# q-optimize/c3

Hardware: AMD Instinct MI355X
Metric: full-gate propagators/s (higher is better)
Workload: dtype c128

## Files before the change

### c3_amd/csrc/c3p_smalld.hip

```cpp
#include <type_traits>

#include <cstdlib>
#include "c3p_common.h"
#include "c3p_kernels.h"
#include "c3p_smalld.h"

#ifdef C3P_SMALLD_PART
#define C3P_SMALLD_HAS(p) (C3P_SMALLD_PART == (p))
#else
#define C3P_SMALLD_HAS(p) 1
#endif

extern __shared__ __attribute__((aligned(16))) double c3p_sd_lds[];

namespace {

template <int D>
struct SD {
  static constexpr int NBI = (D + 1) / 2;
  static constexpr int NJ = (D + 3) / 4;
  static constexpr int W = 4 * NJ + 1;
  static constexpr int MAT = 4 * NBI * W;
  static constexpr int IMG = ((MAT - 12 + 31) / 32) * 32 + 12;
};

__device__ __forceinline__ double mfma4(double a, double b, double c) {
  return __builtin_amdgcn_mfma_f64_4x4x4f64(a, b, c, 0, 0, 0);
}

__device__ __forceinline__ double readfirstlane_f64(double v) {
  int lo = __double2loint(v), hi = __double2hiint(v);
  lo = __builtin_amdgcn_readfirstlane(lo);
  hi = __builtin_amdgcn_readfirstlane(hi);
  return __hiloint2double(hi, lo);
}

typedef __attribute__((address_space(3))) const volatile double c3p_lds_cvd;
__device__ __forceinline__ double lds_ld(const double* p) { return *(c3p_lds_cvd*)p; }

__device__ __forceinline__ double flip_sign(double v, unsigned mask_hi) {
  unsigned long long u = __double_as_longlong(v);
  u ^= ((unsigned long long)mask_hi) << 32;
  return __longlong_as_double(u);
}

__device__ __forceinline__ void wave_sync() {
  __builtin_amdgcn_fence(__ATOMIC_ACQ_REL, "wavefront");
  __builtin_amdgcn_wave_barrier();
}

template <int D>
__device__ __forceinline__ void write_image(const double (&zh)[SD<D>::NBI][SD<D>::NJ], double* img, int woff) {
  using C = SD<D>;
  wave_sync();
#pragma unroll
  for (int I = 0; I < C::NBI; ++I)
#pragma unroll
    for (int J = 0; J < C::NJ; ++J) img[woff + I * 4 * C::W + J * 4] = zh[I][J];
  wave_sync();
}

template <int D>
__device__ __forceinline__ void mm_img(const double* img, int roff, unsigned negmask,
                                       const double (&zb)[SD<D>::NBI][SD<D>::NJ],
                                       double (&acc)[SD<D>::NBI][SD<D>::NJ]) {
  using C = SD<D>;
  double ra[2][C::NBI];
#pragma unroll
  for (int I = 0; I < C::NBI; ++I) ra[0][I] = flip_sign(lds_ld(img + roff + I * 4 * C::W), negmask);
#pragma unroll
  for (int K = 0; K < C::NBI; ++K) {
    if (K + 1 < C::NBI) {
#pragma unroll
      for (int I = 0; I < C::NBI; ++I) ra[(K + 1) & 1][I] = flip_sign(lds_ld(img + roff + I * 4 * C::W + (K + 1) * 2), negmask);
    }
#pragma unroll
    for (int I = 0; I < C::NBI; ++I)
#pragma unroll
      for (int J = 0; J < C::NJ; ++J) acc[I][J] = mfma4(ra[K & 1][I], zb[K][J], acc[I][J]);
    __builtin_amdgcn_sched_barrier(0);
  }
}

struct LanePos {
  int r, b, c;
  int idx16;
};

template <int D>
__device__ __forceinline__ void poly_block(double (&out)[SD<D>::NBI][SD<D>::NJ], double c0, double c1,
                                           double c2, double c3, const double (&X)[SD<D>::NBI][SD<D>::NJ],
                                           const double (&A2)[SD<D>::NBI][SD<D>::NJ],
                                           const double (&A3)[SD<D>::NBI][SD<D>::NJ], int ddelta,
                                           int rhalf) {
  using C = SD<D>;
#pragma unroll
  for (int I = 0; I < C::NBI; ++I)
#pragma unroll
    for (int J = 0; J < C::NJ; ++J) {
      double v = c1 * X[I][J];
      v = fma(c2, A2[I][J], v);
      v = fma(c3, A3[I][J], v);
      if (2 * I - 4 * J >= -1 && 2 * I - 4 * J <= 3) {
        const bool on = (ddelta == 4 * J - 2 * I) && (2 * I + rhalf < D);
        v += on ? c0 : 0.0;
      }
      out[I][J] = v;
    }
}

template <int D>
__device__ __forceinline__ void lincomb6(double (&out)[SD<D>::NBI][SD<D>::NJ], double c0, double cx, double c2,
                                         double c3, double c6, const double (&X)[SD<D>::NBI][SD<D>::NJ],
                                         const double (&A2)[SD<D>::NBI][SD<D>::NJ],
                                         const double (&A3)[SD<D>::NBI][SD<D>::NJ],
                                         const double (&A6)[SD<D>::NBI][SD<D>::NJ], int ddelta, int rhalf) {
  using C = SD<D>;
#pragma unroll
  for (int I = 0; I < C::NBI; ++I)
#pragma unroll
    for (int J = 0; J < C::NJ; ++J) {
      double v = cx * X[I][J];
      v = fma(c2, A2[I][J], v);
      v = fma(c3, A3[I][J], v);
      if (c6 != 0.0) v = fma(c6, A6[I][J], v);
      if (c0 != 0.0 && 2 * I - 4 * J >= -1 && 2 * I - 4 * J <= 3) {
        const bool on = (ddelta == 4 * J - 2 * I) && (2 * I + rhalf < D);
        v += on ? c0 : 0.0;
      }
      out[I][J] = v;
    }
}

template <int D>
struct RD {
  static constexpr int NB = (D + 3) / 4;
};

template <int D>
struct SymTail;
template <int D, bool FULL = false>
__device__ __forceinline__ void sym_fill(double (&m)[RD<D>::NB][RD<D>::NB], int swap_lane);

__device__ __forceinline__ double quad_bcast0(double v) {
  int lo = __double2loint(v), hi = __double2hiint(v);
  lo = __builtin_amdgcn_mov_dpp(lo, 0x00, 0xf, 0xf, true);
  hi = __builtin_amdgcn_mov_dpp(hi, 0x00, 0xf, 0xf, true);
  return __hiloint2double(hi, lo);
}

template <int D>
struct SymTail {
  static constexpr bool ON = (D % 4 == 1) && (RD<D>::NB > 1);
  static constexpr int KM = ON ? RD<D>::NB - 1 : RD<D>::NB;
};

template <int D>
__device__ __forceinline__ constexpr int sym_j0(int I) {
  return I >= SymTail<D>::KM ? I : 0;
}
template <int D, bool FULL>
__device__ __forceinline__ void sym_fill(double (&m)[RD<D>::NB][RD<D>::NB], int swap_lane) {
  constexpr int NB = RD<D>::NB;
  constexpr int ROWS = FULL ? NB : SymTail<D>::KM;
#pragma unroll
  for (int I = 1; I < ROWS; ++I)
#pragma unroll
    for (int J = 0; J < I; ++J) m[I][J] = __shfl(m[J][I], swap_lane);
}
template <int D>
__device__ __forceinline__ void sym_fill_rest(double (&m)[RD<D>::NB][RD<D>::NB], int swap_lane) {
  constexpr int NB = RD<D>::NB;
#pragma unroll
  for (int I = SymTail<D>::KM; I < NB; ++I)
#pragma unroll
    for (int J = 0; J < I; ++J) m[I][J] = __shfl(m[J][I], swap_lane);
}

template <int D>
__device__ __forceinline__ void mm_sym(const double (&za)[RD<D>::NB][RD<D>::NB], const double (&zb)[RD<D>::NB][RD<D>::NB],
                                       double (&acc)[RD<D>::NB][RD<D>::NB], int tail_lane) {
  constexpr int NB = RD<D>::NB;
#pragma unroll
  for (int K = 0; K < SymTail<D>::KM; ++K)
#pragma unroll
    for (int I = 0; I < NB; ++I)
#pragma unroll
      for (int J = I; J < NB; ++J) acc[I][J] = mfma4(za[K][I], zb[K][J], acc[I][J]);
  if constexpr (SymTail<D>::ON) {
    double av[NB], bv[NB];
#pragma unroll
    for (int I = 0; I < NB; ++I) {
      av[I] = quad_bcast0(za[I][NB - 1]);
      bv[I] = __shfl(zb[I][NB - 1], tail_lane);
    }
#pragma unroll
    for (int I = 0; I < NB; ++I)
#pragma unroll
      for (int J = I; J < NB; ++J) acc[I][J] = fma(av[I], bv[J], acc[I][J]);
  }
}
template <int D>
__device__ __forceinline__ void mm_sym2(const double (&za)[RD<D>::NB][RD<D>::NB], const double (&zb1)[RD<D>::NB][RD<D>::NB],
                                        double (&acc1)[RD<D>::NB][RD<D>::NB], const double (&zb2)[RD<D>::NB][RD<D>::NB],
                                        double (&acc2)[RD<D>::NB][RD<D>::NB], int tail_lane) {
  constexpr int NB = RD<D>::NB;
#pragma unroll
  for (int K = 0; K < SymTail<D>::KM; ++K)
#pragma unroll
    for (int I = 0; I < NB; ++I)
#pragma unroll
      for (int J = I; J < NB; ++J) {
        acc1[I][J] = mfma4(za[K][I], zb1[K][J], acc1[I][J]);
        acc2[I][J] = mfma4(za[K][I], zb2[K][J], acc2[I][J]);
      }
  if constexpr (SymTail<D>::ON) {
    double av[NB], bv1[NB], bv2[NB];
#pragma unroll
    for (int I = 0; I < NB; ++I) {
      av[I] = quad_bcast0(za[I][NB - 1]);
      bv1[I] = __shfl(zb1[I][NB - 1], tail_lane);
      bv2[I] = __shfl(zb2[I][NB - 1], tail_lane);
    }
#pragma unroll
    for (int I = 0; I < NB; ++I)
#pragma unroll
      for (int J = I; J < NB; ++J) {
        acc1[I][J] = fma(av[I], bv1[J], acc1[I][J]);
        acc2[I][J] = fma(av[I], bv2[J], acc2[I][J]);
      }
  }
}

template <int D>
__device__ __forceinline__ void mm_symA(const double (&za)[RD<D>::NB][RD<D>::NB], const double (&zb)[RD<D>::NB][RD<D>::NB],
                                        double (&acc)[RD<D>::NB][RD<D>::NB], int row0_lane, double asign) {
  constexpr int NB = RD<D>::NB;
#pragma unroll
  for (int K = 0; K < SymTail<D>::KM; ++K)
#pragma unroll
    for (int I = 0; I < NB; ++I)
#pragma unroll
      for (int J = 0; J < NB; ++J) acc[I][J] = mfma4(za[K][I], zb[K][J], acc[I][J]);
  if constexpr (SymTail<D>::ON) {
    double av[NB], bv[NB];
#pragma unroll
    for (int I = 0; I < NB; ++I) {
      av[I] = asign * quad_bcast0(za[I][NB - 1]);
      bv[I] = __shfl(zb[NB - 1][I], row0_lane);
    }
#pragma unroll
    for (int I = 0; I < NB; ++I)
#pragma unroll
      for (int J = 0; J < NB; ++J) acc[I][J] = fma(av[I], bv[J], acc[I][J]);
  }
}

template <int D>
__device__ __forceinline__ void mm_symfull(const double (&za)[RD<D>::NB][RD<D>::NB], const double (&zb)[RD<D>::NB][RD<D>::NB],
                                           double (&acc)[RD<D>::NB][RD<D>::NB], int tail_lane) {
  constexpr int NB = RD<D>::NB;
#pragma unroll
  for (int K = 0; K < SymTail<D>::KM; ++K)
#pragma unroll
    for (int I = 0; I < NB; ++I)
#pragma unroll
      for (int J = 0; J < NB; ++J) acc[I][J] = mfma4(za[K][I], zb[K][J], acc[I][J]);
  if constexpr (SymTail<D>::ON) {
    double av[NB], bv[NB];
#pragma unroll
    for (int I = 0; I < NB; ++I) {
      av[I] = quad_bcast0(za[I][NB - 1]);
      bv[I] = __shfl(zb[I][NB - 1], tail_lane);
    }
#pragma unroll
    for (int I = 0; I < NB; ++I)
#pragma unroll
      for (int J = 0; J < NB; ++J) acc[I][J] = fma(av[I], bv[J], acc[I][J]);
  }
}

template <int D, bool WITH3, bool UPPER = false>
__device__ __forceinline__ void rcomb(double (&out)[RD<D>::NB][RD<D>::NB], double c0, double c1, double c2, double c3,
                                      const double (&W1)[RD<D>::NB][RD<D>::NB], const double (&W2)[RD<D>::NB][RD<D>::NB],
                                      const double (&W3)[RD<D>::NB][RD<D>::NB], const LanePos& lp) {
  constexpr int NB = RD<D>::NB;
#pragma unroll
  for (int I = 0; I < NB; ++I)
#pragma unroll
    for (int J = (UPPER || I >= SymTail<D>::KM) ? I : 0; J < NB; ++J) {
      double v = c1 * W1[I][J];
      v = fma(c2, W2[I][J], v);
      if constexpr (WITH3) v = fma(c3, W3[I][J], v);
      if (I == J) v += (lp.r == lp.c && 4 * I + lp.r < D) ? c0 : 0.0;
      out[I][J] = v;
    }
}


template <int NC>
struct SMat {
  double m[NC][NC];
  double vr[NC], vc[NC];
  double s;
};
template <int NC>
struct GMat {
  double m[NC][NC];
  double cr[NC], cc[NC], rc[NC];
  double s;
};

template <int NC>
__device__ __forceinline__ void s8_zero(SMat<NC>& a) {
#pragma unroll
  for (int I = 0; I < NC; ++I) {
#pragma unroll
    for (int J = 0; J < NC; ++J) a.m[I][J] = 0.0;
    a.vr[I] = a.vc[I] = 0.0;
  }
  a.s = 0.0;
}

template <int NC>
__device__ __forceinline__ void mm_s8(const SMat<NC>& a, const SMat<NC>& b, SMat<NC>& c) {
#pragma unroll
  for (int I = 0; I < NC; ++I)
#pragma unroll
    for (int J = I; J < NC; ++J) c.m[I][J] = fma(a.vr[I], b.vc[J], c.m[I][J]);
#pragma unroll
  for (int K = 0; K < NC; ++K)
#pragma unroll
    for (int I = 0; I < NC; ++I)
#pragma unroll
      for (int J = I; J < NC; ++J) c.m[I][J] = mfma4(a.m[K][I], b.m[K][J], c.m[I][J]);
  double t[NC], cs = 0.0;
#pragma unroll
  for (int I = 0; I < NC; ++I) {
    t[I] = 0.0;
#pragma unroll
    for (int K = 0; K < NC; ++K) t[I] = fma(a.m[K][I], b.vr[K], t[I]);
    cs = fma(a.vr[I], b.vr[I], cs);
  }
#pragma unroll
  for (int I = 0; I < NC; ++I) c.vr[I] = mfma4(t[I], 1.0, fma(a.vr[I], b.s, c.vr[I]));
  c.s = mfma4(cs, 1.0, fma(a.s, b.s, c.s));
}
template <int NC>
__device__ __forceinline__ void mm_s8x2(const SMat<NC>& a, const SMat<NC>& b1, SMat<NC>& c1, const SMat<NC>& b2, SMat<NC>& c2) {
#pragma unroll
  for (int I = 0; I < NC; ++I)
#pragma unroll
    for (int J = I; J < NC; ++J) {
      c1.m[I][J] = fma(a.vr[I], b1.vc[J], c1.m[I][J]);
      c2.m[I][J] = fma(a.vr[I], b2.vc[J], c2.m[I][J]);
    }
#pragma unroll
  for (int K = 0; K < NC; ++K)
#pragma unroll
    for (int I = 0; I < NC; ++I)
#pragma unroll
      for (int J = I; J < NC; ++J) {
        c1.m[I][J] = mfma4(a.m[K][I], b1.m[K][J], c1.m[I][J]);
        c2.m[I][J] = mfma4(a.m[K][I], b2.m[K][J], c2.m[I][J]);
      }
  double t1[NC], t2[NC], cs1 = 0.0, cs2 = 0.0;
#pragma unroll
  for (int I = 0; I < NC; ++I) {
    t1[I] = t2[I] = 0.0;
#pragma unroll
    for (int K = 0; K < NC; ++K) {
      t1[I] = fma(a.m[K][I], b1.vr[K], t1[I]);
      t2[I] = fma(a.m[K][I], b2.vr[K], t2[I]);
    }
    cs1 = fma(a.vr[I], b1.vr[I], cs1);
    cs2 = fma(a.vr[I], b2.vr[I], cs2);
  }
#pragma unroll
  for (int I = 0; I < NC; ++I) {
    c1.vr[I] = mfma4(t1[I], 1.0, fma(a.vr[I], b1.s, c1.vr[I]));
    c2.vr[I] = mfma4(t2[I], 1.0, fma(a.vr[I], b2.s, c2.vr[I]));
  }
  c1.s = mfma4(cs1, 1.0, fma(a.s, b1.s, c1.s));
  c2.s = mfma4(cs2, 1.0, fma(a.s, b2.s, c2.s));
// ... 932 lines not shown
          mus_i = c3p_phase_add(0.0, mu_i);
        } else {
          RMat Dm, Us, T1, T2, T3;
#pragma unroll
          for (int I = 0; I < NB; ++I)
#pragma unroll
            for (int J = 0; J < NB; ++J) {
              if (J >= sym_j0<D>(I)) Dm[I][J] = Cm[I][J] - acc[I][J];
              Us[I][J] = Ur[I][J] + Ui[I][J];
              T1[I][J] = T2[I][J] = T3[I][J] = 0.0;
            }
          mm_symA<D>(Cm, Ur, T1, row0_lane, 1.0);
          mm_symA<D>(acc, Ui, T2, row0_lane, 1.0);
          mm_symA<D>(Dm, Us, T3, row0_lane, 1.0);
#pragma unroll
          for (int I = 0; I < NB; ++I)
#pragma unroll
            for (int J = 0; J < NB; ++J) {
              Ur[I][J] = T1[I][J] + T2[I][J];
              Ui[I][J] = (T3[I][J] - T1[I][J]) + T2[I][J];
            }
          mus_r += mu_r;
          mus_i = c3p_phase_add(mus_i, mu_i);
        }
      }
      wave_sync();
#pragma unroll
      for (int I = 0; I < NB; ++I)
#pragma unroll
        for (int J = 0; J < NB; ++J) {
          const int i = 4 * I + lp.r, j = 4 * J + lp.c;
          if (2 * i + 1 < 4 * NBI) {
            img[lp.b * IMG + (2 * i) * W + j] = Ur[I][J];
            img[lp.b * IMG + (2 * i + 1) * W + j] = Ui[I][J];
          }
        }
      wave_sync();
#pragma unroll
      for (int I = 0; I < NBI; ++I)
#pragma unroll
        for (int J = 0; J < NJ; ++J) U[I][J] = img[woff + I * 4 * W + J * 4];
      wave_sync();
      img_holds_U = true;
      }
    } else {
    const double* tc = c3p_t18_tab[t18n];
    const double t18_a11 = tc[C3P_I_A11];
    const double t18_a21 = tc[C3P_I_A21];
    const double t18_a31 = tc[C3P_I_A31];
    const double t18_b02 = tc[C3P_I_B02];
    const double t18_b03 = tc[C3P_I_B03];
    const double t18_b11 = tc[C3P_I_B11];
    const double t18_b12 = tc[C3P_I_B12];
    const double t18_b13 = tc[C3P_I_B13];
    const double t18_b21 = tc[C3P_I_B21];
    const double t18_b22 = tc[C3P_I_B22];
    const double t18_b23 = tc[C3P_I_B23];
    const double t18_b24 = tc[C3P_I_B24];
    const double t18_b31 = tc[C3P_I_B31];
    const double t18_b32 = tc[C3P_I_B32];
    const double t18_b33 = tc[C3P_I_B33];
    const double t18_b34 = tc[C3P_I_B34];
    const double t18_b61 = tc[C3P_I_B61];
    const double t18_b62 = tc[C3P_I_B62];
    const double t18_b63 = tc[C3P_I_B63];
    const double t18_b64 = tc[C3P_I_B64];
    auto complex_loop = [&](auto t18_tag) {
    constexpr int VARIANT = decltype(t18_tag)::value;
    constexpr bool T18 = VARIANT == 1;
    for (int t = 0; t < tmax; ++t) {
      const bool act = valid && t < len;
      double sc = act ? scale : 0.0;
      const double muw = act ? 1.0 : 0.0;
      double mu_r, mu_i;
      double X[NBI][NJ];
      int my_s = ps;
      if constexpr (XG) {
        const long m = (long)sample * A.N + n0 + (act ? t : 0);
        {
          const double lim = nrm * scale;
          double scaled = A.meta[m * 4 + 2] * scale;
          while (my_s > 0 && 2.0 * scaled <= lim) {
            scaled *= 2.0;
            --my_s;
          }
          sc = act ? ldexp(1.0, -my_s) : 0.0;
        }
        mu_r = muw * A.meta[m * 4 + 0];
        mu_i = muw * A.meta[m * 4 + 1];
        const double2* src = reinterpret_cast<const double2*>(A.hs) + (long)sample * A.hs_bstride + (long)(n0 + (act ? t : 0)) * D * D;
        const double mine = (lp.r & 1) ? mu_i : mu_r;
#pragma unroll
        for (int I = 0; I < NBI; ++I)
#pragma unroll
          for (int J = 0; J < NJ; ++J) {
            const int row = 2 * I + (lp.r >> 1), col = 4 * J + lp.c;
            const bool in = row < D && col < D;
            const double2 h = src[in ? row * D + col : 0];
            double v = (lp.r & 1) ? fma(A.coef_r, h.y, A.coef_i * h.x) : fma(A.coef_r, h.x, -A.coef_i * h.y);
            v -= (row == col) ? mine : 0.0;
            X[I][J] = in ? sc * v : 0.0;
          }
      } else {
      mu_r = muw * tab[MAT + 0];
      mu_i = muw * tab[MAT + 1];
#pragma unroll
      for (int I = 0; I < NBI; ++I)
#pragma unroll
        for (int J = 0; J < NJ; ++J) X[I][J] = sc * tab[toff + I * 4 * W + J * 4];
      for (int k = 0; k < K; ++k) {
        const double c0 = sg[lp.b * SG + k * A.Lmax + t];
        const double ck = sc * c0;
        const double* tk = tab + (k + 1) * (MAT + 4);
        mu_r = fma(c0, tk[MAT + 0], mu_r);
        mu_i = fma(c0, tk[MAT + 1], mu_i);
#pragma unroll
        for (int I = 0; I < NBI; ++I)
#pragma unroll
          for (int J = 0; J < NJ; ++J) X[I][J] = fma(ck, tk[toff + I * 4 * W + J * 4], X[I][J]);
      }
      }
      write_image<D>(X, img, woff);
      double A2[NBI][NJ], A3[NBI][NJ], P[NBI][NJ];
#pragma unroll
      for (int I = 0; I < NBI; ++I)
#pragma unroll
        for (int J = 0; J < NJ; ++J) A2[I][J] = A3[I][J] = 0.0;
      mm_img<D>(img, roff, negmask, X, A2);
      if constexpr (VARIANT == 2) {
        double y1[NBI][NJ];
        {
          double R[NBI][NJ];
#pragma unroll
          for (int I = 0; I < NBI; ++I)
#pragma unroll
            for (int J = 0; J < NJ; ++J) R[I][J] = fma(c3p_e4n[0], A2[I][J], c3p_e4n[1] * X[I][J]);
          write_image<D>(A2, img, woff);
          mm_img<D>(img, roff, negmask, R, A3);
        }
        {
          double L[NBI][NJ], R[NBI][NJ];
#pragma unroll
          for (int I = 0; I < NBI; ++I)
#pragma unroll
            for (int J = 0; J < NJ; ++J) L[I][J] = fma(c3p_e4n[2], A2[I][J], fma(c3p_e4n[3], X[I][J], A3[I][J]));
          write_image<D>(L, img, woff);
#pragma unroll
          for (int I = 0; I < NBI; ++I)
#pragma unroll
            for (int J = 0; J < NJ; ++J) {
              R[I][J] = fma(c3p_e4n[4], A2[I][J], A3[I][J]);
              y1[I][J] = fma(c3p_e4n[5], A3[I][J], c3p_e4n[6] * A2[I][J]);
            }
          mm_img<D>(img, roff, negmask, R, y1);
        }
        {
          double L[NBI][NJ], R[NBI][NJ];
#pragma unroll
          for (int I = 0; I < NBI; ++I)
#pragma unroll
            for (int J = 0; J < NJ; ++J) L[I][J] = fma(c3p_e4n[7], A2[I][J], fma(c3p_e4n[8], X[I][J], y1[I][J]));
          write_image<D>(L, img, woff);
#pragma unroll
          for (int I = 0; I < NBI; ++I)
#pragma unroll
            for (int J = 0; J < NJ; ++J) {
              R[I][J] = fma(c3p_e4n[9], A3[I][J], fma(c3p_e4n[10], X[I][J], y1[I][J]));
              double v = fma(c3p_e4n[11], y1[I][J], c3p_e4n[12] * A3[I][J]);
              v = fma(c3p_e4n[13], A2[I][J], v);
              v = fma(c3p_e4n[14], X[I][J], v);
              if (2 * I - 4 * J >= -1 && 2 * I - 4 * J <= 3) {
                const bool on = (ddelta == 4 * J - 2 * I) && (2 * I + rhalf < D);
                v += on ? c3p_e4n[15] : 0.0;
              }
              P[I][J] = v;
            }
          mm_img<D>(img, roff, negmask, R, P);
        }
      } else {
      mm_img<D>(img, roff, negmask, A2, A3);
      if constexpr (T18) {
        double A6[NBI][NJ];
#pragma unroll
        for (int I = 0; I < NBI; ++I)
#pragma unroll
          for (int J = 0; J < NJ; ++J) A6[I][J] = 0.0;
        write_image<D>(A3, img, woff);
        mm_img<D>(img, roff, negmask, A3, A6);
        double acc[NBI][NJ];
        {
          double B1[NBI][NJ], B5[NBI][NJ];
          lincomb6<D>(B1, 0.0, t18_a11, t18_a21, t18_a31, 0.0, X, A2, A3, A6, ddelta, rhalf);
          write_image<D>(B1, img, woff);
          lincomb6<D>(B5, 0.0, 0.0, t18_b24, t18_b34, t18_b64, X, A2, A3, A6, ddelta, rhalf);
          lincomb6<D>(acc, t18_b03, t18_b13, t18_b23, t18_b33, t18_b63, X, A2, A3, A6, ddelta, rhalf);
          mm_img<D>(img, roff, negmask, B5, acc);
        }
        {
          double L[NBI][NJ];
          lincomb6<D>(L, t18_b02, t18_b12, t18_b22, t18_b32, t18_b62, X, A2, A3, A6, ddelta, rhalf);
#pragma unroll
          for (int I = 0; I < NBI; ++I)
#pragma unroll
            for (int J = 0; J < NJ; ++J) L[I][J] += acc[I][J];
          write_image<D>(L, img, woff);
        }
        lincomb6<D>(P, 0.0, t18_b11, t18_b21, t18_b31, t18_b61, X, A2, A3, A6, ddelta, rhalf);
        mm_img<D>(img, roff, negmask, acc, P);
      } else {
        {
          double A4[NBI][NJ];
  #pragma unroll
          for (int I = 0; I < NBI; ++I)
  #pragma unroll
            for (int J = 0; J < NJ; ++J) A4[I][J] = 0.0;
          mm_img<D>(img, roff, negmask, A3, A4);
          const int j = pr - 1;
          poly_block<D>(P, c3p_inv_fact[4 * j], c3p_inv_fact[4 * j + 1], c3p_inv_fact[4 * j + 2],
                        c3p_inv_fact[4 * j + 3], X, A2, A3, ddelta, rhalf);
          const double cm = c3p_inv_fact[4 * pr];
  #pragma unroll
          for (int I = 0; I < NBI; ++I)
  #pragma unroll
            for (int J = 0; J < NJ; ++J) P[I][J] = fma(cm, A4[I][J], P[I][J]);
          if (pr > 1) write_image<D>(A4, img, woff);
        }
        for (int j = pr - 2; j >= 0; --j) {
          double acc[NBI][NJ];
          poly_block<D>(acc, c3p_inv_fact[4 * j], c3p_inv_fact[4 * j + 1], c3p_inv_fact[4 * j + 2],
                        c3p_inv_fact[4 * j + 3], X, A2, A3, ddelta, rhalf);
          mm_img<D>(img, roff, negmask, P, acc);
  #pragma unroll
          for (int I = 0; I < NBI; ++I)
  #pragma unroll
            for (int J = 0; J < NJ; ++J) P[I][J] = acc[I][J];
        }
      }
      }
      for (int it = 0; it < ps; ++it) {
        write_image<D>(P, img, woff);
        double acc[NBI][NJ];
#pragma unroll
        for (int I = 0; I < NBI; ++I)
#pragma unroll
          for (int J = 0; J < NJ; ++J) acc[I][J] = 0.0;
        mm_img<D>(img, roff, negmask, P, acc);
        const bool sq = !XG || it < my_s;
#pragma unroll
        for (int I = 0; I < NBI; ++I)
#pragma unroll
          for (int J = 0; J < NJ; ++J) P[I][J] = sq ? acc[I][J] : P[I][J];
      }
      if constexpr (DUS) {
        double sn, cs;
        sincos(mu_i, &sn, &cs);
        const double er = exp(mu_r);
        double* dst = reinterpret_cast<double*>(A.dUs_out) + ((long)sample * A.N + n0 + (act ? t : 0)) * D * D * 2;
        store_plain<D>(P, dst, er * cs, er * sn, nullptr, lp, act);
      }
      if (t == 0) {
#pragma unroll
        for (int I = 0; I < NBI; ++I)
#pragma unroll
          for (int J = 0; J < NJ; ++J) U[I][J] = P[I][J];
        mus_r = mu_r;
        mus_i = c3p_phase_add(0.0, mu_i);
      } else {
        write_image<D>(P, img, woff);
        double acc[NBI][NJ];
#pragma unroll
        for (int I = 0; I < NBI; ++I)
#pragma unroll
          for (int J = 0; J < NJ; ++J) acc[I][J] = 0.0;
        mm_img<D>(img, roff, negmask, U, acc);
#pragma unroll
        for (int I = 0; I < NBI; ++I)
#pragma unroll
          for (int J = 0; J < NJ; ++J) U[I][J] = acc[I][J];
        mus_r += mu_r;
        mus_i = c3p_phase_add(mus_i, mu_i);
      }
    }
    };
    if (t18 == 2)
      complex_loop(std::integral_constant<int, 2>{});
    else if (t18)
      complex_loop(std::integral_constant<int, 1>{});
    else
      complex_loop(std::integral_constant<int, 0>{});
    }
  }
  SD_TICK(tk2);
#ifdef C3P_SD_TIMING
  if (tkl == 0) tkl = tk2;
#endif
  if constexpr (!GIVEN) {
    if (A.fuse) {
      double tr = mus_r, ti = mus_i;
      tr += __shfl_xor(tr, 4);
      tr += __shfl_xor(tr, 8);
      ti = c3p_phase_add(ti, __shfl_xor(ti, 4));
      ti = c3p_phase_add(ti, __shfl_xor(ti, 8));
      const int rrest = roff - lp.b * IMG;
      const int roff1 = ((lp.b + 1) & 3) * IMG + rrest;
      const int roff2 = ((lp.b + 2) & 3) * IMG + rrest;
      double V[NBI][NJ], Wt[NBI][NJ];
      auto fold_slots = [&](const double (&M)[NBI][NJ], bool in_image) {
#pragma unroll
        for (int I = 0; I < NBI; ++I)
#pragma unroll
          for (int J = 0; J < NJ; ++J) V[I][J] = Wt[I][J] = 0.0;
        if (!in_image) write_image<D>(M, img, woff);
        mm_img<D>(img, roff1, negmask, M, V);
        write_image<D>(V, img, woff);
        mm_img<D>(img, roff2, negmask, V, Wt);
      };
      fold_slots(U, img_holds_U);
      SD_TICK(tka);
      const int nW = A.S >> 2;
      const int wq = seg >> 2;
      const double* ph = A.fr_phase ? A.fr_phase + (long)sample * D : nullptr;
      double* dst = reinterpret_cast<double*>(A.final_out) + (long)sample * D * D * 2;
      const int lo = (lp.b * nW) >> 2, hi = ((lp.b + 1) * nW) >> 2;
      const int cnt = hi - lo;
      const int cmax = (nW + 3) >> 2;
      double sn, cs;
      sincos(ti, &sn, &cs);
      double er = 1.0;
      if (__ballot(tr != 0.0) != 0) er = exp(tr);
      SD_TICK(tkb);
      if constexpr (MW) {
        {
          double pr[NBI], pi[NBI];
#pragma unroll
          for (int I = 0; I < NBI; ++I) pr[I] = er * cs, pi[I] = er * sn;
          scale_rows<D>(Wt, pr, pi, lp, V);
        }
        write_image<D>(V, img, woff);
        SD_TICK(tk3);
        double phc[NBI], phs[NBI];
        if (wv == 0) row_phase_factors<D>(ph, lp, phc, phs);
        __syncthreads();
#ifdef C3P_SD_TIMING
        if (blockIdx.x == 7 && lane == 0)
          printf("sd wave %d: slices %d, prologue to the table barrier %lld, behind it %lld, loop ends at %lld (100 MHz ticks after the wave's start); "
                 "layout %lld products %lld phase %lld partial store %lld\n", wv, tmax, tk9 - tk0, tk1 - tk9, tkl - tk0, tk2 - tkl, tka - tk2, tkb - tka, tk3 - tkb);
#endif
        if (wv != 0) return;
        SD_TICK(tk5);
        const int pstride = 4 * IMG + 4 * SG;
        const int woff0 = woff - lp.b * IMG;
#pragma unroll
        for (int I = 0; I < NBI; ++I)
#pragma unroll
          for (int J = 0; J < NJ; ++J) {
            const int row = 2 * I + (lp.r >> 1), col = 4 * J + lp.c;
            const double idv = (row < D && row == col && (lp.r & 1) == 0) ? 1.0 : 0.0;
            U[I][J] = cnt > 0 ? img[lo * pstride + woff0 + I * 4 * W + J * 4] : idv;
          }
        for (int t = 1; t < cmax; ++t) {
          const bool act = t < cnt;
          double acc[NBI][NJ];
#pragma unroll
          for (int I = 0; I < NBI; ++I)
#pragma unroll
            for (int J = 0; J < NJ; ++J) acc[I][J] = 0.0;
          mm_img<D>(img, (act ? lo + t : 0) * pstride + rrest, negmask, U, acc);
#pragma unroll
          for (int I = 0; I < NBI; ++I)
#pragma unroll
            for (int J = 0; J < NJ; ++J) U[I][J] = act ? acc[I][J] : U[I][J];
        }
        SD_TICK(tk6);
        fold_slots(U, false);
        SD_TICK(tk7);
        store_plain<D>(Wt, dst, 1.0, 0.0, ph, lp, lp.b == 0, phc, phs);
#ifdef C3P_SD_TIMING
        SD_TICK(tk4);
        if (blockIdx.x == 0 && threadIdx.x == 0)
          printf("sd timing (100 MHz ticks): tables %lld signals %lld prologue %lld loop %lld fold4+store %lld barrier %lld level1 %lld fold2 %lld store %lld total %lld\n", tk8 - tk0, tk9 - tk8, tk1 - tk0, tk2 - tk1, tk3 - tk2, tk5 - tk3, tk6 - tk5, tk7 - tk6, tk4 - tk7, tk4 - tk0);
#endif
        return;
      }
      if (nW == 1) {
        store_plain<D>(Wt, dst, er * cs, er * sn, ph, lp, valid && lp.b == 0);
        return;
      }
      {
        double* pdst = reinterpret_cast<double*>(A.seg_out) + ((long)sample * nW + wq) * D * D * 2;
        store_plain<D, true>(Wt, pdst, er * cs, er * sn, nullptr, lp, valid && lp.b == 0);
      }
      asm volatile("s_waitcnt vmcnt(0)" ::: "memory");
      int old = 0;
      if (lane == 0)
        old = __hip_atomic_fetch_add(A.counters + sample, 1, __ATOMIC_RELAXED, __HIP_MEMORY_SCOPE_AGENT);
      old = __builtin_amdgcn_readfirstlane(old);
      if (old != nW - 1) return;
      if (lane == 0) A.counters[sample] = 0;
      __builtin_amdgcn_fence(__ATOMIC_ACQUIRE, "agent");
      const double* base = reinterpret_cast<const double*>(A.seg_out) + ((long)sample * nW + lo) * D * D * 2;
      double Pn[NBI][NJ];
      auto fetch = [&](double (&P)[NBI][NJ], int t) {
        const bool act = t < cnt;
        const double* src = base + (long)(act ? t : 0) * D * D * 2;
#pragma unroll
        for (int I = 0; I < NBI; ++I)
#pragma unroll
          for (int J = 0; J < NJ; ++J) {
            const int row = 2 * I + (lp.r >> 1), col = 4 * J + lp.c;
            const bool in = row < D && col < D;
            const double idv = (in && row == col && (lp.r & 1) == 0) ? 1.0 : 0.0;
            P[I][J] = (act && in) ? src[(row * D + col) * 2 + (lp.r & 1)] : idv;
          }
      };
      fetch(U, 0);
      if (cmax > 1) fetch(Pn, 1);
      for (int t = 1; t < cmax; ++t) {
        double P[NBI][NJ];
#pragma unroll
        for (int I = 0; I < NBI; ++I)
#pragma unroll
          for (int J = 0; J < NJ; ++J) P[I][J] = Pn[I][J];
        if (t + 1 < cmax) fetch(Pn, t + 1);
        {
          double acc[NBI][NJ];
#pragma unroll
          for (int I = 0; I < NBI; ++I)
#pragma unroll
            for (int J = 0; J < NJ; ++J) acc[I][J] = 0.0;
          write_image<D>(P, img, woff);
          mm_img<D>(img, roff, negmask, U, acc);
#pragma unroll
          for (int I = 0; I < NBI; ++I)
#pragma unroll
            for (int J = 0; J < NJ; ++J) U[I][J] = acc[I][J];
        }
      }
      fold_slots(U, false);
      store_plain<D>(Wt, dst, 1.0, 0.0, ph, lp, lp.b == 0);
      return;
    }
  }
  double sn, cs;
  sincos(mus_i, &sn, &cs);
  const double er = exp(mus_r);
  double* dst = reinterpret_cast<double*>(A.seg_out) + (long)cc * D * D * 2;
  const double* ph = A.fr_phase ? A.fr_phase + (long)sample * D : nullptr;
  store_plain<D>(U, dst, er * cs, er * sn, ph, lp, valid);
}

template <int D>
__global__ void __launch_bounds__(64) smalld_prep_kernel(PrepArgs P) {
  using C = SD<D>;
  constexpr int MAT = C::MAT, W = C::W;
  __shared__ double g[D * D * 2];
  __shared__ double colsum[D];
  __shared__ double mu[2];
  const int tid = threadIdx.x;
  const int ti = blockIdx.x % (1 + P.K);
  const int sample = blockIdx.x / (1 + P.K);
  if (P.counters != nullptr && blockIdx.x == 0)
    for (int e = tid; e < P.ncounters; e += 64) P.counters[e] = 0;
  const int Dh = P.Dh;
  const cplx* h = (ti == 0) ? P.h0 + (long)sample * P.h0_bstride
                            : P.hks + (long)sample * P.hks_bstride + (long)(ti - 1) * Dh * Dh;
  for (int e = tid; e < D * D; e += 64) {
    const int row = e / D, col = e - row * D;
    cplx v;
    if (!P.lindblad) {
      const cplx x = h[e];
      v = cmake(x.y * P.dt, -x.x * P.dt);
    } else {
      const int i = row / Dh, j = row - i * Dh, k = col / Dh, l = col - k * Dh;
      v = (ti == 0) ? P.clp[(long)sample * P.clp_bstride + e] : cmake(0, 0);
      if (j == l) {
        const cplx x = h[i * Dh + k];
        v.x += x.y;
        v.y -= x.x;
      }
      if (i == k) {
        const cplx x = h[l * Dh + j];
        v.x -= x.y;
        v.y += x.x;
      }
      v = cscale(v, P.dt);
    }
    const int eo = P.conjT ? col * D + row : e;
    g[2 * eo] = v.x;
    g[2 * eo + 1] = P.conjT ? -v.y : v.y;
  }
  __syncthreads();
  if (tid == 0) {
    double tr = 0, ti2 = 0;
    for (int i = 0; i < D; ++i) {
      tr += g[2 * (i * D + i)];
      ti2 += g[2 * (i * D + i) + 1];
    }
    mu[0] = 0.0;
    mu[1] = ti2 / D;
  }
  __syncthreads();
  if (tid < D) {
    g[2 * (tid * D + tid)] -= mu[0];
    g[2 * (tid * D + tid) + 1] -= mu[1];
  }
  __syncthreads();
  if (tid < D) {
    double s = 0;
    for (int i = 0; i < D; ++i) s += hypot(g[2 * (i * D + tid)], g[2 * (i * D + tid) + 1]);
    colsum[tid] = s;
  }
  __syncthreads();
  double* out = P.tables + ((long)sample * (1 + P.K) + ti) * (MAT + 4);
  for (int e = tid; e < MAT; e += 64) {
    const int rho = e / W, col = e - rho * W;
    const int i = rho >> 1, p = rho & 1;
    out[e] = (i < D && col < D) ? g[2 * (i * D + col) + p] : 0.0;
  }
  if (tid == 0) {
    double nrm = 0;
    for (int j = 0; j < D; ++j) nrm = fmax(nrm, colsum[j]);
    out[MAT + 0] = mu[0];
    out[MAT + 1] = mu[1];
    out[MAT + 2] = nrm;
    double remax = 0, asym = 0, rsk = 0;
    for (int e = 0; e < D * D; ++e) {
      const int i = e / D, j = e - i * D;
      remax = fmax(remax, fabs(g[2 * e]));
      asym = fmax(asym, fabs(g[2 * e + 1] - g[2 * (j * D + i) + 1]));
      rsk = fmax(rsk, fabs(g[2 * e] + g[2 * (j * D + i)]));
    }
    if (asym > 1e-14 * nrm) remax = fmax(remax, asym);
    if (remax > 0.0 && fmax(asym, rsk) <= 1e-14 * nrm) remax = -remax;
    out[MAT + 3] = P.lindblad ? 1.0 : remax;
  }
}

template <int D>
hipError_t launch_chain_t(const SmallArgs& A, hipStream_t st) {
  using C = SD<D>;
  const long nchains = (long)A.B * A.S;
  const unsigned grid = (unsigned)((nchains + 3) / 4);
  size_t lds = 0;
  const size_t cs_tail1 = (1 + A.K) * SD_CSW <= 4 * C::IMG ? 0 : (size_t)(1 + A.K) * SD_CSW;
  if (A.mode == C3P_MODE_GIVEN || A.mode == C3P_MODE_EXPM)
    lds = (size_t)(4 * C::IMG) * sizeof(double);
  else
    lds = (size_t)((1 + A.K) * (C::MAT + 4) + 4 * C::IMG + 4 * ((A.K * A.Lmax) | 1) + cs_tail1) * sizeof(double);
  const bool split81 = (D == 9 || D == 5) && !c3p_opt_on(C3P_OPT_no_split81);
  const int krows = A.K + ((split81 && A.K > 0) ? 1 : 0);
  if (lds > 60 * 1024) return hipErrorInvalidValue;
  if (A.mode == C3P_MODE_EXPM) {
    if (A.dUs_out)
      C3P_LAUNCH((smalld_chain_kernel<D, false, true, true>), dim3(grid), dim3(64), lds, st, A);
    else
      C3P_LAUNCH((smalld_chain_kernel<D, false, false, true>), dim3(grid), dim3(64), lds, st, A);
  } else if (A.mode == C3P_MODE_GIVEN)
    C3P_LAUNCH((smalld_chain_kernel<D, true, false>), dim3(grid), dim3(64), lds, st, A);
  else if (A.dUs_out)
    C3P_LAUNCH((smalld_chain_kernel<D, false, true>), dim3(grid), dim3(64), lds, st, A);
  else {
    const int nW = A.S >> 2;
    const size_t wstride = (size_t)(4 * C::IMG + 4 * ((krows * A.Lmax) | 1));
    const size_t tail_mw = std::max((size_t)nW * D * D * 2, (size_t)(1 + A.K) * SD_CSW);
    const size_t lds_mw = (size_t)((1 + A.K) * (C::MAT + 4) + nW * wstride + tail_mw) * sizeof(double);
    const bool mw = A.fuse && (A.S & 3) == 0 && (nW == 2 || nW == 4 || nW == 8) && (long)A.B * nW <= 2048 &&
                    lds_mw * (8 / nW) <= (size_t)156 * 1024 && !c3p_opt_on(C3P_OPT_no_mw);
    if (mw) {
      SmallArgs A2 = A;
      if (nW == 8 && A.N >= 4 * A.S) {
        int skew = ((D == 9 || D == 5) && !c3p_opt_on(C3P_OPT_no_split81)) ? (D == 9 ? 704 : 700) : 640, skew_c = 640;
        if (c3p_opt(C3P_OPT_mw_skew) >= 0) skew = skew_c = (int)c3p_opt(C3P_OPT_mw_skew);
        if (skew > 500 && skew < 900) {
          const int h = A.S / 2;
          int lmax = 0;
          auto split = [&](int per_mille) {
            int La = (int)(((long)A.N * per_mille) / (500L * A.S));
            if (La < 1) La = 1;
            if ((long)h * La > A.N - h) La = (A.N - h) / h;
            const long rest = (long)A.N - (long)h * La;
            const int Lb = (int)((rest + h - 1) / h);
            lmax = std::max(lmax, std::max(La, Lb));
            return La;
          };
          A2.seg_long = split(skew);
          A2.seg_long_c = (skew_c > 500 && skew_c < 900 && skew_c != skew) ? split(skew_c) : 0;
          A2.Lmax = lmax;
        }
      }
      const size_t wstride2 = (size_t)(4 * C::IMG + 4 * ((krows * A2.Lmax) | 1));
      const size_t lds_mw2 = (size_t)((1 + A2.K) * (C::MAT + 4) + nW * wstride2 + tail_mw) * sizeof(double);
      if (lds_mw2 > (size_t)156 * 1024) A2 = A;
      const size_t lds_use = A2.seg_long > 0 ? lds_mw2 : lds_mw;
      auto kern = smalld_chain_kernel<D, false, false, false, true>;
      if constexpr (D == 9 || D == 5) {
        if (!c3p_opt_on(C3P_OPT_no_split81)) kern = smalld_chain_kernel<D, false, false, false, true, true>;
      }
      if (lds_use > 64 * 1024) {
        hipError_t e = hipFuncSetAttribute(reinterpret_cast<const void*>(kern), hipFuncAttributeMaxDynamicSharedMemorySize, (int)lds_use);
        if (e != hipSuccess) return e;
      }
      C3P_LAUNCH(kern, dim3((unsigned)A.B), dim3(64 * nW), lds_use, st, A2);
    } else {
      auto kern1 = smalld_chain_kernel<D, false, false>;
      if constexpr (D == 9 || D == 5) {
        if (!c3p_opt_on(C3P_OPT_no_split81)) kern1 = smalld_chain_kernel<D, false, false, false, false, true>;
      }
      const size_t lds1 = (size_t)((1 + A.K) * (C::MAT + 4) + 4 * C::IMG + 4 * ((krows * A.Lmax) | 1) + cs_tail1) * sizeof(double);
      if (lds1 > 60 * 1024) return hipErrorInvalidValue;
      C3P_LAUNCH(kern1, dim3(grid), dim3(64), lds1, st, A);
    }
  }
  return hipGetLastError();
}

template <int D>
__device__ __forceinline__ void write_image_H(const double (&zh)[SD<D>::NBI][SD<D>::NJ], double* img, const LanePos& lp) {
  using C = SD<D>;
// ... 1052 lines not shown
```

Before: 2.635 million.

## Split fold-slot matrix products across lane blocks as a tree reduction

```diff
diff --git a/c3_amd/csrc/c3p_smalld.hip b/c3_amd/csrc/c3p_smalld.hip
--- a/c3_amd/csrc/c3p_smalld.hip
+++ b/c3_amd/csrc/c3p_smalld.hip
@@ -80,6 +80,105 @@
       for (int J = 0; J < C::NJ; ++J) acc[I][J] = mfma4(ra[K & 1][I], zb[K][J], acc[I][J]);
     __builtin_amdgcn_sched_barrier(0);
   }
+}
+
+struct SDTile {
+  int I, J;
+  bool on;
+};
+
+template <int D>
+constexpr int sd_split_tasks(int nb) {
+  return (SD<D>::NBI * SD<D>::NJ + nb - 1) / nb;
+}
+
+template <int D>
+constexpr SDTile sd_split_deal(int nb, int blk, int task) {
+  constexpr int NBI = SD<D>::NBI, NJ = SD<D>::NJ;
+  const int per = sd_split_tasks<D>(nb);
+  const int full = NBI / per, rem = NBI % per;
+  if (blk < NJ * full) return SDTile{(blk % full) * per + task, blk / full, true};
+  const int idx = (blk - NJ * full) * per + task;
+  if (rem == 0 || idx >= NJ * rem) return SDTile{0, 0, false};
+  return SDTile{full * per + idx % rem, idx / rem, true};
+}
+
+template <int D>
+constexpr bool sd_split_deal_ok(int nb) {
+  constexpr int NBI = SD<D>::NBI, NJ = SD<D>::NJ;
+  int seen[NBI][NJ] = {};
+  for (int blk = 0; blk < nb; ++blk)
+    for (int t = 0; t < sd_split_tasks<D>(nb); ++t) {
+      const SDTile s = sd_split_deal<D>(nb, blk, t);
+      if (s.I < 0 || s.I >= NBI || s.J < 0 || s.J >= NJ) return false;
+      if (s.on) ++seen[s.I][s.J];
+    }
+  for (int I = 0; I < NBI; ++I)
+    for (int J = 0; J < NJ; ++J)
+      if (seen[I][J] != 1) return false;
+  return true;
+}
+#define C3P_SD_DEAL_OK(D) static_assert(sd_split_deal_ok<D>(2) && sd_split_deal_ok<D>(4), "split product: every output tile exactly once")
+C3P_SD_DEAL_OK(2); C3P_SD_DEAL_OK(3); C3P_SD_DEAL_OK(4); C3P_SD_DEAL_OK(5); C3P_SD_DEAL_OK(6); C3P_SD_DEAL_OK(7);
+C3P_SD_DEAL_OK(8); C3P_SD_DEAL_OK(9); C3P_SD_DEAL_OK(10); C3P_SD_DEAL_OK(11); C3P_SD_DEAL_OK(12);
+#undef C3P_SD_DEAL_OK
+static_assert(sd_split_deal<9>(4, 2, 3).I == 3 && sd_split_deal<9>(4, 2, 3).J == 2 && sd_split_deal<9>(4, 3, 1).I == 4 &&
+                  sd_split_deal<9>(4, 3, 1).J == 1 && !sd_split_deal<9>(4, 3, 3).on,
+              "D = 9 over four blocks: a column each on blocks 0 .. 2, the last row on block 3");
+
+template <int D, int NB>
+__device__ __forceinline__ void split_offsets(int blk, int (&aoff)[sd_split_tasks<D>(NB)], int (&coff)[sd_split_tasks<D>(NB)],
+                                              int (&joff)[sd_split_tasks<D>(NB)], bool (&on)[sd_split_tasks<D>(NB)]) {
+  using C = SD<D>;
+#pragma unroll
+  for (int t = 0; t < sd_split_tasks<D>(NB); ++t) {
+    int I = sd_split_deal<D>(NB, 0, t).I, J = sd_split_deal<D>(NB, 0, t).J;
+    bool o = sd_split_deal<D>(NB, 0, t).on;
+#pragma unroll
+    for (int q = 1; q < NB; ++q) {
+      I = blk == q ? sd_split_deal<D>(NB, q, t).I : I;
+      J = blk == q ? sd_split_deal<D>(NB, q, t).J : J;
+      o = blk == q ? sd_split_deal<D>(NB, q, t).on : o;
+    }
+    aoff[t] = I * 4 * C::W;
+    joff[t] = J * 4;
+    coff[t] = I * 4 * C::W + J * 4;
+    on[t] = o;
+  }
+}
+
+template <int D, int NB>
+__device__ __forceinline__ void mm_split(const double* a, double* bc, unsigned negmask, int blk) {
+  using C = SD<D>;
+  constexpr int NT = sd_split_tasks<D>(NB);
+  int aoff[NT], coff[NT], joff[NT];
+  bool on[NT];
+  split_offsets<D, NB>(blk, aoff, coff, joff, on);
+  double ra[2][NT], rb[2][NT], acc[NT];
+#pragma unroll
+  for (int t = 0; t < NT; ++t) {
+    ra[0][t] = flip_sign(lds_ld(a + aoff[t]), negmask);
+    rb[0][t] = lds_ld(bc + joff[t]);
+    acc[t] = 0.0;
+  }
+#pragma unroll
+  for (int K = 0; K < C::NBI; ++K) {
+    if (K + 1 < C::NBI) {
+#pragma unroll
+      for (int t = 0; t < NT; ++t) {
+        ra[(K + 1) & 1][t] = flip_sign(lds_ld(a + aoff[t] + (K + 1) * 2), negmask);
+        rb[(K + 1) & 1][t] = lds_ld(bc + (K + 1) * 4 * C::W + joff[t]);
+      }
+    }
+#pragma unroll
+    for (int t = 0; t < NT; ++t) acc[t] = mfma4(ra[K & 1][t], rb[K & 1][t], acc[t]);
+    __builtin_amdgcn_sched_barrier(0);
+  }
+  wave_sync();
+#pragma unroll
+  for (int t = 0; t < NT; ++t)
+    if (on[t]) bc[coff[t]] = acc[t];
+  wave_sync();
 }
 
 struct LanePos {
@@ -1618,18 +1717,29 @@
       ti = c3p_phase_add(ti, __shfl_xor(ti, 4));
       ti = c3p_phase_add(ti, __shfl_xor(ti, 8));
       const int rrest = roff - lp.b * IMG;
-      const int roff1 = ((lp.b + 1) & 3) * IMG + rrest;
-      const int roff2 = ((lp.b + 2) & 3) * IMG + rrest;
       double V[NBI][NJ], Wt[NBI][NJ];
+      constexpr bool FOLD_SPLIT = MW && NBI * NJ > 2 && D <= 9;
       auto fold_slots = [&](const double (&M)[NBI][NJ], bool in_image) {
-#pragma unroll
-        for (int I = 0; I < NBI; ++I)
-#pragma unroll
-          for (int J = 0; J < NJ; ++J) V[I][J] = Wt[I][J] = 0.0;
         if (!in_image) write_image<D>(M, img, woff);
-        mm_img<D>(img, roff1, negmask, M, V);
-        write_image<D>(V, img, woff);
-        mm_img<D>(img, roff2, negmask, V, Wt);
+        if constexpr (FOLD_SPLIT) {
+          const int wrest = woff - lp.b * IMG;
+          mm_split<D, 2>(img + ((lp.b & 2) + 1) * IMG + rrest, img + (lp.b & 2) * IMG + wrest, negmask, lp.b & 1);
+          mm_split<D, 4>(img + 2 * IMG + rrest, img + wrest, negmask, lp.b);
+#pragma unroll
+          for (int I = 0; I < NBI; ++I)
+#pragma unroll
+            for (int J = 0; J < NJ; ++J) Wt[I][J] = img[wrest + I * 4 * W + J * 4];
+        } else {
+          const int roff1 = ((lp.b + 1) & 3) * IMG + rrest;
+          const int roff2 = ((lp.b + 2) & 3) * IMG + rrest;
+#pragma unroll
+          for (int I = 0; I < NBI; ++I)
+#pragma unroll
+            for (int J = 0; J < NJ; ++J) V[I][J] = Wt[I][J] = 0.0;
+          mm_img<D>(img, roff1, negmask, M, V);
+          write_image<D>(V, img, woff);
+          mm_img<D>(img, roff2, negmask, V, Wt);
+        }
       };
       fold_slots(U, img_holds_U);
       SD_TICK(tka);
```

Measured after the change: 2.663 million, median of 6. 1.1% higher.
